# CasperTheCat/Vermilion

Measured on AMD Instinct MI355X. Metric: Mrays/sec (primary+secondary), 1920x1080 Sponza, higher is better.
Workload: dtype f32

## Files before the change

### vermilion_amd/csrc/api_render.inc

```
namespace {

Tuning make_tuning(const vmx_scene *sc, const vmx_opts *o) {
    Tuning tn;
    tn.refill_min = o->reserved[3] ? o->reserved[3] : 8u;
    tn.refill_primary = o->reserved[3] ? o->reserved[3] : 64u;
    tn.shade_min = o->reserved[4] ? o->reserved[4] : 16u;
    tn.leaf_min = 0xFFFFFFFFu;
    tn.sort_mode = o->reserved[5];
    tn.two_phase = false;
    tn.sorted = false;
    tn.bounce_records = false;
    tn.pool = false;
    tn.guide = false;
    const uint32_t cap = o->reserved[6];
    tn.lds_entries = std::min(sc->dev.stack_entries, cap ? cap : 10u);
    tn.lds_primary = std::min(sc->dev.stack_entries, cap ? cap : (uint32_t)VMX_LDS_PRIMARY);
    tn.lds_bounce = std::min(sc->dev.stack_entries, cap ? cap : 9u);
    tn.tail_threshold = o->reserved[2] ? o->reserved[2] : (16u << 20);
    return tn;
}


int bind_stack(vmx_scene *sc, const Tuning &tn, uint32_t entries, uint32_t grid, uint64_t items, WorkDev &wk, bool guided = false) {
    const uint64_t per_lane = items / ((uint64_t)grid * kPathsBlock);
// ... 248 lines not shown
    uint32_t smax = (uint32_t)std::max<uint64_t>(1, max_paths / npix);
    if (opts->samples_per_batch) smax = opts->samples_per_batch;
    smax = std::min(smax, fr.kmax);
    const size_t n_pad_cap = ((size_t)npix + 63u) & ~(size_t)63u;
    if (!opts->samples_per_batch && !legacy) {
        const size_t per_path = 16 + 64 + 8 + 16 + 12  + (sc->dev.tex ? 16 : 0) + (tn.sort_mode ? 12 : 0) + (fr.elide_dead ? 5 : 0) + 32 + (tn.guide ? 4 : 0) ;
        size_t free_b = 0, total_b = 0;
        HIP_TRY(hipMemGetInfo(&free_b, &total_b));
        const size_t held = ws.rayA.n + ws.state.n + ws.hit.n + ws.rad.n + ws.thr.n + (ws.ids[0].n + ws.ids[1].n + ws.ids[2].n) * 4 +
                            (ws.sort_keys[0].n + ws.sort_keys[1].n + ws.ids_sorted.n) * 4 + ws.out_rec.n + ws.live_ids.n * 4 +
                            ws.guide_fb.n * 4;
        job.mem_budget = (uint64_t)((free_b + held) / 10 * 9);
        if (const char *e = std::getenv("VMX_MEM_BUDGET_MB")) {
            const uint64_t cap = std::strtoull(e, nullptr, 10) << 20;
            if (cap) job.mem_budget = std::min(job.mem_budget, cap);
        }
        const uint64_t fixed = (uint64_t)npix * 48 + ((uint64_t)sc->n_inner * 512 + (uint64_t)sc->ntris * 64) + (64ull << 20);
        const uint64_t fit = job.mem_budget > fixed ? (job.mem_budget - fixed) / per_path : 0;
        const uint32_t s_fit = (uint32_t)std::min<uint64_t>(std::max<uint64_t>(1, fit / n_pad_cap), fr.kmax);
        if (s_fit < smax) smax = s_fit;
    }
    if (fr.early_stop) smax = std::min(smax, fr.nmin + 1 + (fr.quarter ? fr.kmax / fr.quarter - 1u : 0u));
    if (!fr.early_stop && !opts->samples_per_batch) {
        const uint32_t npass = (fr.kmax + smax - 1) / smax;
        smax = (fr.kmax + npass - 1) / npass;
    }
    job.smax = job.smax_alloc = smax;

    HIP_TRY((hipError_t)query_paths_blocks_per_cu(kPathsBlock, (kPathsBlock / 64) * (tn.lds_entries + 1) * 512, count, &job.rb, tn.guide));
    if (job.rb < 1) return fail(VMX_ERR_HIP, "kernel does not fit on a CU (LDS stack too deep?)");

    job.n_pad_max = (npix + 63u) & ~63u;
    const uint32_t tiles8_max = (((job.n_pad_max + sc->block - 1) / sc->block) + 7u) & ~7u;
    job.sub_cap = ((tiles8_max * smax) / kSubQueues + 2) * sc->block;
    job.sub_cap = job.sub_cap + job.sub_cap / 4 + 4096;
    tn.bounce_records = split_any && !tn.two_phase && !count && !tn.pool && fr.r2scale == 10.0f;
    if (split_any) {
        HIP_TRY((hipError_t)query_trace_q_blocks_per_cu(kPathsBlock, (kPathsBlock / 64) * (tn.lds_primary + 1) * 512, count, false,
                                                        tn.sorted, fr.elide_dead != 0, &job.tb));
        HIP_TRY((hipError_t)query_trace_q_blocks_per_cu(kPathsBlock, (kPathsBlock / 64) * (tn.lds_bounce + 1) * 512, count, true,
                                                        tn.sorted || tn.bounce_records, false, &job.tbb, tn.guide));
        if (job.tb < 1 || job.tbb < 1) return fail(VMX_ERR_HIP, "trace kernel does not fit on a CU");
        job.tbb = ab_bounce_blocks(job.tbb);
    }
    job.elide = split_any && fr.elide_dead;
    job.claims_on = split_any && !count && !job.elide && !(opts->reserved[0] & 0x800u) &&
                    (pipeline == 4 || (uint64_t)job.n_pad_max * smax >= kHybridPaths);
    job.fuse_on = job.claims_on && !tn.two_phase && !tn.sorted && !(opts->reserved[0] & 0x1000u);
    job.lists_on = job.claims_on && !(opts->reserved[0] & 0x2000u);
    job.live_words_max = ((size_t)job.n_pad_max * smax + 63) / 64;
    if (job.elide) job.live_tmp_bytes = live_compact_tmp_bytes((uint32_t)job.live_words_max);
    if (pixels->ensure(npix)) return fail(VMX_ERR_NOMEM, "hipMalloc failed for the per-pixel state");
    job.n_active = npix;
    return VMX_OK;
}

int render_init_pixels(vmx_scene *sc, RenderJob &job) {
    Workspace &ws = sc->ws;
    const uint32_t W = job.fr.width, rows = job.fr.local_rows;
    if (ws.order_w != W || ws.order_rows != rows) {
        tile_order(W, rows, ws.order);
        ws.order_w = W, ws.order_rows = rows;
    }
    HIP_TRY(hipMemcpyAsync(job.pixels->active[0].p, ws.order.data(), (size_t)job.npix * 4, hipMemcpyHostToDevice, job.s));
    LAUNCH_TRY(launch_init_pixels(PixelStateDev{job.pixels->accum.p, job.pixels->count.p, job.pixels->cursor.p}, job.npix, job.s));
    job.launches++;
    job.initialised = true;
    return VMX_OK;
}

constexpr uint32_t kClaimMinSamples = 64;
uint32_t claim_min_samples() {
#ifdef VMX_AB_KERNELS
    if (const char *e = std::getenv("VMX_CLAIM_MIN_SPP")) {
        const unsigned long v = std::strtoul(e, nullptr, 10);
        if (v) return (uint32_t)std::min<unsigned long>(v, 0xFFFFFFFFul);
    }
#endif
    return kClaimMinSamples;
}

int build_claims(vmx_scene *sc, const FrameDev &fr, const Tuning &tn, uint32_t npix, bool lists, hipStream_t s) {
    Workspace &ws = sc->ws;
    if (ws.claims.ensure((size_t)npix + 1)) return fail(VMX_ERR_NOMEM, "hipMalloc failed for the pixel claims");
    if (lists && ws.claim_lists.ensure((size_t)npix * kListWords)) return fail(VMX_ERR_NOMEM, "hipMalloc failed for the claim lists");
    WorkDev wk;
    std::memset(&wk, 0, sizeof(wk));
    wk.cam_inner = ws.cam_inner.p, wk.cam_tris = ws.cam_inner.p + std::max<size_t>(sc->n_inner, 1) * 64 * 8;
    const uint32_t tiles = ((fr.width + 7u) / 8u) * ((fr.local_rows + 7u) / 8u);
    LaunchCfg cfg = paths_cfg(sc, tn.lds_primary, (uint64_t)tiles * 64, 8);
    int rc = bind_stack(sc, tn, tn.lds_primary, cfg.grid, (uint64_t)tiles * 64, wk);
    if (rc) return rc;
    HIP_TRY(hipMemsetAsync(ws.claims.p + npix, 0, 4, s));
    LAUNCH_TRY(launch_pixel_claims(sc->dev, fr, wk, ws.claims.p, lists ? ws.claim_lists.p : nullptr, ws.claims.p + npix, cfg, s));
    return VMX_OK;
}

int nee_launch_cfg(vmx_scene *sc, const Tuning &tn, uint64_t items, bool rays, WorkDev &wk, LaunchCfg &cfg, bool budgeted = false) {
    int blocks = 0;
    HIP_TRY((hipError_t)query_nee_blocks_per_cu(kPathsBlock, (kPathsBlock / 64) * (tn.lds_entries + 1) * 512, rays, &blocks, budgeted));
    if (blocks < 1) return fail(VMX_ERR_HIP, "kernel does not fit on a CU (LDS stack too deep?)");
    cfg = paths_cfg(sc, tn.lds_entries, items, blocks);
    return bind_stack(sc, tn, tn.lds_entries, cfg.grid, items, wk);
}

int render_bind(vmx_scene *sc, RenderJob &job, uint32_t run_samples) {
    Workspace &ws = sc->ws;
    const FrameDev &fr = job.fr;
    const Tuning &tn = job.tn;
    const uint32_t smax = job.smax, n_pad_max = job.n_pad_max;
    hipStream_t s = job.s;
    if (job.nee) {
        if (ws.heads.ensure(kSubQueues * 32) || ws.rad.ensure((size_t)n_pad_max * smax * 16) || ws.next_count.ensure(32) ||
            ws.counters.ensure(1))
            return fail(VMX_ERR_NOMEM, "hipMalloc failed for the render workspace");
        job.px = PixelStateDev{job.pixels->accum.p, job.pixels->count.p, job.pixels->cursor.p};
        job.claims = job.claim_lists = nullptr;
        return VMX_OK;
    }
    if (job.split_any) {
        int rc = ensure_paths(sc, (size_t)n_pad_max * smax, job.pa, job.qi);
        if (rc == VMX_ERR_NOMEM && smax > 1 && !job.opts.samples_per_batch)
            return fail(VMX_ERR_NOMEM, "hipMalloc failed for the path arrays although " + std::to_string(job.mem_budget >> 20) +
                                           " MB were reported free: set VMX_MEM_BUDGET_MB or vmx_opts.reserved[1] (paths per pass)");
        if (rc) return rc;
    }
    else if (job.legacy) {
        int rc = ab_bind_legacy(sc, job);
        if (rc) return rc;
    }
    if (ws.heads.ensure(kSubQueues * 32)) return fail(VMX_ERR_NOMEM, "work heads");
    if (ws.rad_mask.ensure(((size_t)n_pad_max * smax + 63) / 64 + 8)) return fail(VMX_ERR_NOMEM, "hipMalloc failed for the radiance mask");
    if (job.split_any) job.pa.rad_mask = ws.rad_mask.p;
    if (job.split_any && tn.two_phase) {
        const size_t words = job.live_words_max + 2048;
        const size_t tmp = live_compact_tmp_bytes((uint32_t)words);
        if (ws.full_mask.ensure(words + 8) || ws.full_u32.ensure(2 * words + 16) || ws.full_tmp.ensure(tmp + 256))
            return fail(VMX_ERR_NOMEM, "hipMalloc failed for the two-phase shading lists");
        ws.full_words = words, ws.full_tmp_bytes = tmp;
    }
    if (job.split_any && (tn.sorted || tn.bounce_records)) {
        const size_t waves = (size_t)sc->num_cus * ((size_t)std::max(job.tb, job.tbb) + (tn.guide ? kGuideFallbackBlocks : 0u)) * (kPathsBlock / 64);
        ws.out_capacity = (size_t)n_pad_max * smax + waves * 256 + 1024;
        if (ws.out_capacity > 0xFFFFFFFFull) return fail(VMX_ERR_INVALID, "pass too large for the sorted ray records");
        if (ws.out_rec.ensure(ws.out_capacity * (tn.sorted ? 32 : 16)) || ws.out_count.ensure(32))
            return fail(VMX_ERR_NOMEM, "hipMalloc failed for the ray records");
    }
    if (job.split_any) {
        if (ws.guide_ctr.ensure(2) || (tn.guide && (ws.guide_fb.ensure((size_t)job.qi[0].sub_capacity * kSubQueues) ||
                                                    ws.guide_fb_count.ensure(32) || ws.guide_heads.ensure(32))))
            return fail(VMX_ERR_NOMEM, "hipMalloc failed for the guide tree's fallback list");
    }
    if (job.elide) {
        if (ws.live_mask.ensure(job.live_words_max + 8) || ws.live_u32.ensure(2 * job.live_words_max + 16) ||
            ws.live_ids.ensure((size_t)n_pad_max * smax + 64) || ws.live_tmp.ensure(job.live_tmp_bytes + 256))
            return fail(VMX_ERR_NOMEM, "hipMalloc failed for the live-path list");
    }
    if (ws.rad.ensure((size_t)n_pad_max * smax * 16) || ws.next_count.ensure(32) || ws.counters.ensure(1) ||
        (tn.guide && ws.guide_fused_ctr.ensure(2)))
        return fail(VMX_ERR_NOMEM, "hipMalloc failed for the render workspace");
    job.px = PixelStateDev{job.pixels->accum.p, job.pixels->count.p, job.pixels->cursor.p};
    if (job.split_any) {
        const size_t n_inner = std::max<size_t>(sc->n_inner, 1);
        if (ws.cam_inner.ensure(n_inner * 64 * 8 + (size_t)sc->ntris * 64))
            return fail(VMX_ERR_NOMEM, "hipMalloc failed for the camera tables");
        LAUNCH_TRY(launch_camera_tables(sc->dev, sc->n_inner, fr.px, fr.py, fr.pz, ws.cam_inner.p,
                                        ws.cam_inner.p + n_inner * 64 * 8, s));
        job.launches++;
    }
    job.claims = job.claim_lists = nullptr;
    if (job.claims_on) {
        uint32_t expect = fr.early_stop ? std::min(fr.kmax, fr.nmin + 1 + (fr.quarter ? fr.kmax / fr.quarter - 1u : 0u)) : fr.kmax;
        if (run_samples) expect = std::min(expect, run_samples);
        if (expect >= claim_min_samples()) {
            int rc = timed_begin(ws, job.timed, s, -1, VMX_K_OTHER);
            if (rc) return rc;
            if ((rc = build_claims(sc, fr, tn, job.npix, job.lists_on, s))) return rc;
// ... 639 lines not shown
```

### vermilion_amd/csrc/vmx_host.h

```cpp
namespace {

thread_local std::string g_err;

int fail(int code, const std::string &msg) {
    g_err = msg;
    return code;
}

#define HIP_TRY(expr)                                                                              \
    do {                                                                                           \
        hipError_t e_ = (expr);                                                                    \
        if (e_ != hipSuccess)                                                                      \
            return fail(VMX_ERR_HIP, std::string(#expr) + ": " + hipGetErrorString(e_));           \
    } while (0)

#define LAUNCH_TRY(expr)                                                                           \
    do {                                                                                           \
        int e_ = (expr);                                                                           \
        if (e_ != 0)                                                                               \
            return fail(VMX_ERR_HIP, std::string(#expr) + ": " + hipGetErrorString((hipError_t)e_)); \
    } while (0)

const vmx_sphere kReferenceSpheres[8] = {
    {{15.f, 140.f, 25.f}, 3.5f, {0.f * 15.f, .5f * 15.f, 1.0f * 15.f}, VMX_SPHERE_EMIT, {-55.f, 350.f, -150.f}, -1.f},
// ... 26 lines not shown
        if (p) (void)hipFree(p);
        p = nullptr;
        n = 0;
        hipError_t e = hipMalloc((void **)&p, std::max<size_t>(count, 1) * sizeof(T));
        if (e != hipSuccess) return (int)e;
        n = count;
        return 0;
    }
    void release() {
        if (p) (void)hipFree(p);
        p = nullptr;
        n = 0;
    }
};
static_assert(!std::is_copy_constructible<DevBuf<float>>::value, "DevBuf owns its memory: it moves, it is never copied");

struct NoCopy {
    NoCopy() = default;
    NoCopy(const NoCopy &) = delete;
    NoCopy &operator=(const NoCopy &) = delete;
};

struct DevStream : NoCopy {
    hipStream_t s = nullptr;
    ~DevStream() { if (s) (void)hipStreamDestroy(s); }
    operator hipStream_t() const { return s; }
};

struct EventPool : NoCopy {
    std::vector<hipEvent_t> ev;
    size_t used = 0;
    ~EventPool() { for (auto e : ev) (void)hipEventDestroy(e); }
    hipEvent_t get() {
        if (used == ev.size()) {
            hipEvent_t e;
            if (hipEventCreate(&e) != hipSuccess) return nullptr;
            ev.push_back(e);
        }
        return ev[used++];
    }
    void reset() { used = 0; }
};

struct Fence : NoCopy {
    hipEvent_t ev = nullptr;
    bool recorded = false;
    ~Fence() { if (ev) (void)hipEventDestroy(ev); }
    int wait(hipStream_t s) const {
        if (recorded) HIP_TRY(hipStreamWaitEvent(s, ev, 0));
        return VMX_OK;
    }
    int record(hipStream_t s) {
        if (!ev) HIP_TRY(hipEventCreateWithFlags(&ev, hipEventDisableTiming));
        HIP_TRY(hipEventRecord(ev, s));
        recorded = true;
        return VMX_OK;
    }
    int sync() const {
        if (recorded) HIP_TRY(hipEventSynchronize(ev));
        return VMX_OK;
    }
};

struct PixelBufs {
    DevBuf<unsigned char> accum;
    DevBuf<unsigned int> count, cursor, active[2];
    int ensure(size_t npix) {
        return accum.ensure(npix * 16) || count.ensure(npix) || cursor.ensure(npix) || active[0].ensure(npix) || active[1].ensure(npix);
    }
};

struct Workspace {
    DevBuf<unsigned char> queue_planes[2];
    DevBuf<unsigned int> queue_counts;
    DevBuf<unsigned int> heads;
    DevBuf<unsigned char> overflow_stack;
    DevBuf<unsigned char> rayA, state, hit, thr;
    DevBuf<unsigned int> ids[3], id_counts;
    DevBuf<unsigned int> sort_keys[2], ids_sorted;
    DevBuf<unsigned char> sort_tmp;
    DevBuf<unsigned char> cam_inner;
    DevBuf<unsigned int> claims;
    DevBuf<unsigned int> claim_lists;
    DevBuf<unsigned int> unclaimed, claimed_slots, unclaimed_u32;
    DevBuf<unsigned long long> unclaimed_mask;
    DevBuf<unsigned char> unclaimed_tmp;
    size_t unclaimed_words = 0, unclaimed_tmp_bytes = 0;
    DevBuf<unsigned int> walk_slots, walk_u32;
    DevBuf<unsigned long long> walk_mask;
    DevBuf<unsigned char> rad;
    DevBuf<unsigned long long> rad_mask;
    DevBuf<unsigned long long> live_mask;
    DevBuf<unsigned int> live_u32, live_ids;
    DevBuf<unsigned char> live_tmp;
    DevBuf<unsigned long long> full_mask;
    DevBuf<unsigned int> full_u32;
    DevBuf<unsigned char> full_tmp;
    size_t full_words = 0, full_tmp_bytes = 0;
    DevBuf<unsigned char> out_rec;
    DevBuf<unsigned int> out_count;
    size_t out_capacity = 0;
    DevBuf<unsigned int> guide_fb, guide_fb_count, guide_heads;
    DevBuf<unsigned long long> guide_ctr;
    DevBuf<unsigned long long> guide_fused_ctr;
    uint64_t guide_entries = 0;
    PixelBufs pixels;
    DevBuf<unsigned int> next_count;
    DevBuf<DevCounters> counters;
    DevBuf<float> out;
    std::vector<unsigned int> order;
    uint32_t order_w = 0, order_rows = 0;
    EventPool events;
};

}

#define VMX_OPAQUE __attribute__((visibility("hidden")))

struct vmx_scene {
    int device = 0;
    int num_cus = 0;
    DevStream stream;
    HostBvh bvh;
    LbvhDevice lbvh;
    bool device_built = false;
    uint32_t builder = VMX_BVH_REFERENCE;
    std::atomic<bool> flat_ready{true};
    bool flat_topology = true;
    uint32_t n_inner = 0;
    uint32_t ntris = 0, leaf_size = 4;
    std::vector<vmx_sphere> spheres;
    DevBuf<unsigned char> d_geom;
    DevBuf<AttrRecord> d_attrs;
    DevBuf<SphereDev> d_spheres;
    DevBuf<float> d_tex, d_tex1;
    uint32_t n_textures = 0;
    SceneDev dev{};
    std::mutex mu;
    Workspace ws;
    uint32_t block = 256;
    float bounds_lo[3] = {0, 0, 0}, bounds_hi[3] = {1, 1, 1};
    vmx_timings timings{};
    uint64_t fused_paths = 0;
    uint64_t list_settled = 0;
    uint64_t guide_settled = 0, guide_fallback = 0;
    uint64_t guide_entries = 0;
    uint64_t guide_fused_settled = 0, guide_fused_fallback = 0;
    struct VMX_OPAQUE Guide {
        std::shared_ptr<const HostBvh> host;
        const unsigned char *base = nullptr;
        uint32_t off = 0;
        size_t bytes = 0;
        uint32_t tri_off = 0, root_ref = 0, stack_entries = 0;
        float scene_max = 0.f;
        bool valid = false;
    } guide;
    struct QueryWs {
        DevBuf<unsigned int> head;
        DevBuf<unsigned char> overflow_stack;
        Fence done;
        uint32_t lds_entries = 0, overflow_entries = 0;
        uint32_t grid[2][kQueryModes] = {};
        uint32_t stack_entries = 0;
        DevBuf<unsigned char> albedo_rec;
    } qws;
    struct VMX_OPAQUE UpdateState {
// ... 213 lines not shown
```

### vermilion_amd/csrc/vmx_kernels.h

```cpp
#pragma once
#include <stdint.h>
#include "vmx_device.h"

namespace vmx {

constexpr uint32_t kSubQueues = 16;

struct QueueDev {
    void *planes;
    unsigned int *counts;
    uint32_t capacity;
    uint32_t sub_capacity;
};

struct PixelStateDev {
    void *accum;
    unsigned int *count;
    unsigned int *cursor;
};

struct PathArrays {
    void *rayA;
    void *state;
    void *hit;
// ... 58 lines not shown
    uint32_t fb_capacity;
    unsigned int *fb_ids;
    unsigned int *fb_count;
    unsigned long long *ctr;
    DevCounters *overflow;
};

struct GuidePathsDev {
    uint32_t off;
    uint32_t tri_off;
    uint32_t root_ref;
    float scene_max;
    unsigned long long *ctr;
};

struct QueryDev {
    const float *o, *d;
    const float *tmax;
    uint32_t n;
    uint32_t reserve;
    uint32_t refill_min;
    uint32_t lds_entries;
    uint32_t overflow_entries;
    uint32_t sample;
    void *overflow_stack;
    unsigned int *head;
    int32_t *tri_id;
    float *t;
    uint8_t *hit;
};

struct LaunchCfg {
    uint32_t grid;
    uint32_t block;
    uint32_t lds_bytes;
};

int launch_trace(const SceneDev &sc, const float *o, const float *d, uint32_t n, int32_t *tri_id,
                 float *t, DevCounters *counters, bool count, LaunchCfg cfg, void *stream);
int launch_raycast(const SceneDev &sc, const float *o, const float *d, uint32_t n, void *out_rayhit,
                   LaunchCfg cfg, void *stream);
int launch_primary_ids(const SceneDev &sc, const FrameDev &fr, uint32_t k, int32_t *tri_id, float *t,
                       LaunchCfg cfg, void *stream);

constexpr uint32_t kQueryCastRays = 3, kQueryCastCamera = 4, kQueryModes = 5;
int launch_query(const SceneDev &sc, const QueryDev &q, uint32_t mode, bool quad, LaunchCfg cfg, void *stream);
int query_query_blocks_per_cu(uint32_t block, uint32_t lds_bytes, uint32_t mode, bool quad, int *blocks);
int launch_raycast_query(const SceneDev &sc, const QueryDev &q, const FrameDev &fr, bool camera, bool quad, void *out,
                         LaunchCfg cfg, uint32_t finish_grid, void *stream);

struct RefitItem {
    uint32_t ref, dst;
};
constexpr uint32_t kRefitRoot = 0xFFFFFFFFu;
int launch_update_records(uint32_t ntris, const float *pos, const float *nrm, const float *uv, void *tris, void *attrs,
                          void *stream);
int launch_refit_level(const RefitItem *items, uint32_t n, const float *pos, const void *tris, void *inner,
                       float *root_box, void *stream);
int launch_attrs_by_id(uint32_t ntris, const void *tris, const void *attrs, float *nrm, float *uv, void *stream);

int launch_trig(const float *x, uint32_t n, float *cs, float *sn, void *stream);

int launch_init_pixels(PixelStateDev px, uint32_t npix, void *stream);
int launch_zero_u32(unsigned int *p, uint32_t n, void *stream);
#ifdef VMX_AB_KERNELS
int launch_primary(const SceneDev &sc, const FrameDev &fr, const unsigned int *active,
                   uint32_t n_active, uint32_t samples, PixelStateDev px, QueueDev qout, void *rad,
                   DevCounters *counters, bool count, bool loop_to_end, LaunchCfg cfg, void *stream);
int launch_radiance_init(const float *o, const float *d, uint32_t n, uint64_t seed, QueueDev qout,
                         void *stream);
int launch_bounce(const SceneDev &sc, float r2scale, uint32_t libm_double, QueueDev qin, uint32_t max_chunks, QueueDev qout,
                  void *rad, DevCounters *counters, bool count, bool loop_to_end, bool first_step,
                  LaunchCfg cfg, void *stream);
int query_blocks_per_cu(uint32_t block, uint32_t lds_bytes, bool count, int *primary_blocks, int *bounce_blocks);
int launch_trace_pool(const SceneDev &sc, const WorkDev &wk, PathArrays pa, LaunchCfg cfg, void *stream);
int query_trace_pool(uint32_t block, uint32_t pool_slots, uint32_t lds_levels, uint32_t *lds_bytes, int *blocks);
#endif
int launch_paths(const SceneDev &sc, const FrameDev &fr, const WorkDev &wk, PixelStateDev px, void *rad,
                 DevCounters *counters, bool count, LaunchCfg cfg, void *stream, const GuidePathsDev *guide = nullptr);
int query_paths_blocks_per_cu(uint32_t block, uint32_t lds_bytes, bool count, int *blocks, bool guide = false);
int launch_camera_tables(const SceneDev &sc, uint32_t n_inner, float ox, float oy, float oz, void *cam_inner,
                         void *cam_tris, void *stream);
int launch_pixel_claims(const SceneDev &sc, const FrameDev &fr, const WorkDev &wk, unsigned int *claims, unsigned int *lists, unsigned int *n_claimed,
                        LaunchCfg cfg, void *stream);
int launch_raygen(const SceneDev &sc, const FrameDev &fr, const WorkDev &wk, PixelStateDev px, PathArrays pa, void *stream);
int launch_raygen_live(const SceneDev &sc, const FrameDev &fr, const WorkDev &wk, PixelStateDev px, PathArrays pa, void *stream);
size_t live_compact_tmp_bytes(uint32_t nwords);
int launch_live_compact(const unsigned long long *live_mask, const unsigned int *live_cnt, uint32_t nwords,
                        unsigned int *offs, unsigned int *ids, unsigned int *count, void *tmp, size_t tmp_bytes, void *stream);
int launch_slot_lists(const unsigned long long *mask, const unsigned int *cnt, uint32_t nwords, uint32_t n_active, unsigned int *offs,
                      unsigned int *unclaimed, unsigned int *claimed, unsigned int *counts, void *tmp, size_t tmp_bytes, void *stream);
int launch_unclaimed_words(const unsigned int *active, uint32_t n_active, uint32_t n_pad, const unsigned int *claims,
                           unsigned long long *mask, unsigned int *cnt, void *stream);
int launch_walk_words(const unsigned int *active, uint32_t n_active, uint32_t n_pad, const unsigned int *claims,
                      const unsigned int *lists, unsigned long long *mask, unsigned int *cnt, void *stream);
int launch_trace_q(const SceneDev &sc, const FrameDev &fr, const WorkDev &wk, PixelStateDev px, PathArrays pa,
                   DevCounters *counters, bool count, bool from_queue, LaunchCfg cfg, void *stream, const GuideDev *guide = nullptr,
                   unsigned int *visits = nullptr);
int query_trace_q_blocks_per_cu(uint32_t block, uint32_t lds_bytes, bool count, bool from_queue, bool sorted, bool live, int *blocks,
                                bool guide = false);
int launch_shade(const SceneDev &sc, const FrameDev &fr, const WorkDev &wk, PixelStateDev px, PathArrays pa,
                 IdQueue qout, uint32_t max_chunks, DevCounters *counters, bool from_queue, void *stream);
int launch_shade_ends(const SceneDev &sc, const FrameDev &fr, const WorkDev &wk, PathArrays pa, unsigned long long *full_mask,
                      unsigned int *full_cnt, uint32_t max_chunks, DevCounters *counters, bool from_queue, void *stream);
int launch_tail(const SceneDev &sc, const FrameDev &fr, const WorkDev &wk, PathArrays pa, DevCounters *counters,
                bool count, LaunchCfg cfg, void *stream, const GuidePathsDev *guide = nullptr);
int launch_radiance_init_ids(const float *o, const float *d, uint32_t n, uint64_t seed, PathArrays pa,
                             IdQueue qout, void *stream);
int launch_resolve(const FrameDev &fr, const unsigned int *active, uint32_t n_active, uint32_t samples,
                   bool pixel_major, const void *rad, const unsigned long long *rad_mask, PixelStateDev px, unsigned int *next_active,
                   unsigned int *next_count, float *out_rgbaz, DevCounters *counters, void *stream, bool moments = false);
int launch_list_words(const unsigned int *list, uint32_t n, const unsigned char *select, const unsigned int *cursor, uint32_t kmax,
                      unsigned long long *mask, unsigned int *cnt, void *stream);
int launch_list_compact(const unsigned long long *mask, const unsigned int *cnt, uint32_t nwords, unsigned int *offs,
                        const unsigned int *src, unsigned int *dst, unsigned int *count, void *tmp, size_t tmp_bytes, void *stream);
struct SamplingPass {
    uint32_t width, height;
    uint32_t kmax, min_samples, radius;
    float threshold, floor;
    PixelStateDev px;
};
int launch_sampling_error(const SamplingPass &a, float *error, float *variance, void *stream);
int launch_sampling_select(const SamplingPass &a, unsigned char *select, unsigned int *count, void *stream);
int launch_bruteforce(const SceneDev &sc, const FrameDev &fr, const unsigned int *order, uint32_t npix, uint32_t flags,
                      float *out, DevCounters *counters, void *longs , unsigned int *long_count,
                      const WorkDev &stack , LaunchCfg cfg, void *stream);
int launch_bruteforce_long(const SceneDev &sc, const FrameDev &fr, uint32_t flags, float *out, DevCounters *counters,
                           const void *longs, const unsigned int *long_count, uint32_t count, const WorkDev &stack,
                           LaunchCfg cfg, void *stream);
int launch_preview(PixelStateDev px, uint32_t npix, uint32_t kmax, const float *finished, float *out_rgbaz, void *rgba8,
                   void *stream);
struct FilterSrc {
    const float *frame;
    PixelStateDev px;
    const float *finished;
    uint32_t kmax;
};
struct FilterPass {
    uint32_t width, height;
    uint32_t step;
    uint32_t squarings;
    float isc2, kz;
    const void *guide;
    FilterSrc src;
    const void *in_plane;
    void *out_plane;
    float *out_rgbaz;
    void *rgba8;
    bool first, last;
    float sl2;
    const void *albedo;
};
static_assert(sizeof(FilterPass) == 128, "FilterPass: a member moved (the kernels' argument offsets would)");
int launch_filter_guide(const void *rayhit, uint32_t npix, void *guide, void *stream);
int launch_atrous(const FilterPass &pass, void *stream);
int launch_demod_divide(const FilterPass &pass, void *stream);
int launch_variance_pack(const FilterPass &pass, const float *variance, void *stream);
int launch_atrous_var(const FilterPass &pass, void *stream);
struct UpsamplePass {
    uint32_t width, height, low_width, low_height;
    uint32_t squarings;
    float sigma_depth;
    const void *guide_low, *guide_full;
    const float *low;
    float *out_rgbaz;
    void *rgba8;
};
// ... 89 lines not shown
```

### vermilion_amd/csrc/vmx_kernels.hip

```cpp
#include <hip/hip_runtime.h>
#include <math.h>
#include <algorithm>
#include <stdint.h>

#include "vmx_kernels.h"
#include "pixel_claim.h"
#include "guide_walk.h"
#include <type_traits>

#ifndef VMX_CAM_BATCH
#define VMX_CAM_BATCH 16
#endif
#ifndef VMX_TRACE_WAVES_PER_SIMD
#define VMX_TRACE_WAVES_PER_SIMD 7
#endif


namespace vmx {
__device__ __forceinline__ float luminance(float r, float g, float b);
namespace {

constexpr float kInf = __builtin_huge_valf();

struct Cnt {
// ... 1369 lines not shown
            } else if ((int)cur < 0) {
                if (COUNT) {
                    if (P.depth == 0) c0.tris++;
                    else c1.tris++;
                }
                float dist;
                const bool hit = tri_test(q0, q1, q2.x, P.ox, P.oy, P.oz, P.dx, P.dy, P.dz, dist);
                if (hit && dist < best) {
                    if (GUIDE) second = best, cut = toff != 0 ? dist * kGwCut : dist;
                    best = dist;
                    slot = (int)(cur & kLeafStartMask);
                } else if (GUIDE && hit) {
                    second = fminf(second, dist);
                }
                cur = leaf_advance(cur);
            }
            if (cur == kPop) {
                const uint32_t ref = pop_to_next(stk, ovf, lds_entries, sp, GUIDE ? cut : best);
                cur = ref == kBottom ? kIdle : ref;
            }
        };
        if (__builtin_amdgcn_ballot_w64(exact && cur != kIdle) != 0) {
#pragma unroll 1
            for (int act = 0; act < 8; ++act) step(std::true_type{});
        } else {
#pragma unroll 1
            for (int act = 0; act < 8; ++act) step(std::false_type{});
        }
    }
    tally_flush<COUNT>(ctr, tl, c0, c1);
    if (GUIDE && lane == 0) {
        if (n_settled) atomicAdd(&gd.ctr[0], (unsigned long long)n_settled);
        if (n_fallback) atomicAdd(&gd.ctr[1], (unsigned long long)n_fallback);
    }
}





__global__ void k_camera_tables(SceneDev sc, uint32_t n_inner, float ox, float oy, float oz,
                                float4 *__restrict__ cam_inner, float4 *__restrict__ cam_tris) {
    const float4 *__restrict__ inner = (const float4 *)sc.inner;
    const float4 *__restrict__ tris = (const float4 *)sc.tris;
    const uint32_t total = n_inner + sc.ntris;
    for (uint32_t i = blockIdx.x * blockDim.x + threadIdx.x; i < total; i += gridDim.x * blockDim.x) {
        if (i < n_inner) {
            const float4 q0 = inner[i * 4], q1 = inner[i * 4 + 1], q2 = inner[i * 4 + 2], q3 = inner[i * 4 + 3];
            const float l0x = q0.x - ox, l0y = q0.y - oy, l0z = q0.z - oz, h0x = q0.w - ox, h0y = q1.x - oy, h0z = q1.y - oz;
            const float l1x = q1.z - ox, l1y = q1.w - oy, l1z = q2.x - oz, h1x = q2.y - ox, h1y = q2.z - oy, h1z = q2.w - oz;
            for (uint32_t o = 0; o < 8; ++o) {
                const bool sx = o & 1u, sy = o & 2u, sz = o & 4u;
                float4 *rec = cam_inner + ((size_t)o * n_inner + i) * 4;
                rec[0] = make_float4(sx ? h0x : l0x, sy ? h0y : l0y, sz ? h0z : l0z, sx ? l0x : h0x);
                rec[1] = make_float4(sy ? l0y : h0y, sz ? l0z : h0z, sx ? h1x : l1x, sy ? h1y : l1y);
                rec[2] = make_float4(sz ? h1z : l1z, sx ? l1x : h1x, sy ? l1y : h1y, sz ? l1z : h1z);
                rec[3] = q3;
            }
        } else {
            const uint32_t t = i - n_inner;
            const float4 a = tris[t * 3], b = tris[t * 3 + 1], c = tris[t * 3 + 2];
            const float e1x = a.w, e1y = b.x, e1z = b.y, e2x = b.z, e2y = b.w, e2z = c.x;
            const float tx = ox - a.x, ty = oy - a.y, tz = oz - a.z;
            float qx, qy, qz;
            cross3(tx, ty, tz, e1x, e1y, e1z, qx, qy, qz);
            const float cdot = dot3(e2x, e2y, e2z, qx, qy, qz);
            cam_tris[t * 4] = make_float4(e1x, e1y, e1z, e2x);
            cam_tris[t * 4 + 1] = make_float4(e2y, e2z, tx, ty);
            cam_tris[t * 4 + 2] = make_float4(tz, qx, qy, qz);
            cam_tris[t * 4 + 3] = make_float4(cdot, c.y, 0.f, 0.f);
        }
    }
}

struct ClaimStack {
    uint2 *stk, *ovf;
    int lds_entries;
    __device__ __forceinline__ void put(int i, uint32_t ref, float near) { stack_push(stk, ovf, lds_entries, i, make_uint2(ref, __float_as_uint(near))); }
    __device__ __forceinline__ void get(int i, uint32_t &ref, float &near) const {
        const uint2 e = stack_pop(stk, ovf, lds_entries, i);
        ref = e.x, near = __uint_as_float(e.y);
    }
};
__global__ void __launch_bounds__(256)
k_pixel_claims(SceneDev sc, FrameDev fr, const float *__restrict__ cam_inner, const float *__restrict__ cam_tris,
               unsigned int *__restrict__ claims, unsigned int *__restrict__ lists, unsigned int *n_claimed, uint32_t lds_levels,
               uint32_t overflow_entries, void *overflow_stack) {
    extern __shared__ uint2 lds_stack[];
    const uint32_t lane = threadIdx.x & 63u, wave = threadIdx.x >> 6;
    ClaimStack stk;
    stk.stk = lds_stack + (size_t)wave * (lds_levels + 1) * 64 + lane;
    stk.ovf = (uint2 *)overflow_stack + ((size_t)(blockIdx.x * (blockDim.x >> 6) + wave) * overflow_entries) * 64 + lane;
    stk.lds_entries = (int)lds_levels;
    PcFilm fm;
    for (int i = 0; i < 9; ++i) fm.m[i] = fr.m[i];
    fm.width = fr.width, fm.height = fr.height, fm.sensor_x = fr.sensor_x, fm.sensor_y = fr.sensor_y, fm.film_dist = fr.film_dist;
    const uint32_t tiles_x = (fr.width + 7u) / 8u, tiles = tiles_x * ((fr.local_rows + 7u) / 8u);
    uint32_t n = 0;
    for (uint32_t tile = blockIdx.x * (blockDim.x >> 6) + wave; tile < tiles; tile += gridDim.x * (blockDim.x >> 6)) {
        const uint32_t ty = tile / tiles_x, tx = tile - ty * tiles_x;
        const uint32_t x = tx * 8u + (lane & 7u), y = ty * 8u + (lane >> 3);
        if (x < fr.width && y < fr.local_rows) {
            const uint32_t lp = y * fr.width + x;
            uint32_t c;
            if (lists) {
                uint32_t l[kListWords];
                c = pc_pixel_claim_and_list(fm, global_pixel(fr, lp), cam_inner, cam_tris, sc.root_ref, stk,
                                            (int)(lds_levels + overflow_entries), l);
                ((uint4 *)lists)[lp] = make_uint4(l[0], l[1], l[2], l[3]);
            } else {
                c = pc_pixel_claim(fm, global_pixel(fr, lp), cam_inner, cam_tris, sc.root_ref, stk, (int)(lds_levels + overflow_entries));
            }
            claims[lp] = c;
            n += c != kClaimNone ? 1u : 0u;
        }
    }
    n = wave_sum(n);
    if (lane == 0 && n) atomicAdd(n_claimed, n);
}

__global__ void __launch_bounds__(256)
k_unclaimed_words(const unsigned int *__restrict__ active, uint32_t n_active, uint32_t n_pad, const unsigned int *__restrict__ claims,
                  unsigned long long *__restrict__ mask, unsigned int *__restrict__ cnt) {
    for (uint32_t s_idx = blockIdx.x * blockDim.x + threadIdx.x; s_idx < n_pad; s_idx += gridDim.x * blockDim.x) {
        const bool un = s_idx < n_active && claims[active[s_idx]] == kClaimNone;
        const unsigned long long bits = __builtin_amdgcn_ballot_w64(un);
        if ((threadIdx.x & 63u) == 0) mask[s_idx >> 6] = bits, cnt[s_idx >> 6] = (uint32_t)__popcll(bits);
    }
}

__global__ void __launch_bounds__(256)
k_walk_words(const unsigned int *__restrict__ active, uint32_t n_active, uint32_t n_pad, const unsigned int *__restrict__ claims,
             const unsigned int *__restrict__ lists, unsigned long long *__restrict__ mask, unsigned int *__restrict__ cnt) {
    for (uint32_t s_idx = blockIdx.x * blockDim.x + threadIdx.x; s_idx < n_pad; s_idx += gridDim.x * blockDim.x) {
        bool walk = false;
        if (s_idx < n_active) {
            const uint32_t lp = active[s_idx];
            walk = claims[lp] == kClaimNone && lists[(size_t)lp * kListWords] == kClaimNone;
        }
        const unsigned long long bits = __builtin_amdgcn_ballot_w64(walk);
        if ((threadIdx.x & 63u) == 0) mask[s_idx >> 6] = bits, cnt[s_idx >> 6] = (uint32_t)__popcll(bits);
    }
}

template <int LIVE, bool LISTS = false>
__global__ void __launch_bounds__(256)
k_raygen(SceneDev sc, FrameDev fr, WorkDev wk, PixelStateDev px, PathArrays pa) {
    static_assert(!LISTS || !LIVE, "list pixels are settled in the plain form");
    const uint32_t total = wk.samples * wk.n_pad;
    [[maybe_unused]] uint32_t n_listed = 0;
    if (wk.pixel_major && (wk.samples & 63u) == 0) {
        const uint32_t lane = threadIdx.x & 63u;
        const uint32_t waves = gridDim.x * (blockDim.x >> 6);
        const uint32_t chunks = wk.samples >> 6;
        const bool listed = !LIVE && wk.unclaimed != nullptr;
        const uint32_t units = listed ? *wk.unclaimed_count : wk.n_pad;
        for (uint32_t unit = (uint32_t)__builtin_amdgcn_readfirstlane((int)(blockIdx.x * (blockDim.x >> 6) + (threadIdx.x >> 6)));
             unit < units; unit += waves) {
            const uint32_t s_idx = listed ? wk.unclaimed[unit] : unit;
            const uint32_t pid_base = s_idx * wk.samples;
            if (s_idx < wk.n_active) {
                const uint32_t lp = wk.active[s_idx];
                const uint32_t pixel = global_pixel(fr, lp);
                const PixelKey pk = rng_pixel_key(fr.seed, pixel);
                const bool lights = (LIVE || fr.camera_bits) && pixel_may_reach_a_light(sc, fr, pixel);
                const uint32_t cur = px.cursor[lp];
                const uint32_t k0 = cur & ~kCursorStrided, kstep = (cur & kCursorStrided) ? fr.quarter : 1u;
                typedef uint32_t u32x4 __attribute__((ext_vector_type(4)));
                [[maybe_unused]] u32x4 lrec = {kClaimNone, kClaimNone, kClaimNone, kClaimNone};
                if constexpr (LISTS) lrec = ((const __attribute__((address_space(4))) u32x4 *)(uintptr_t)wk.claim_lists)[lp];
                for (uint32_t ch = 0; ch < chunks; ++ch) {
                    const uint32_t j = ch * 64u + lane;
                    const uint32_t k = (fr.lead != 0 && j >= fr.lead) ? (j - fr.lead + 1u) * fr.quarter : k0 + j * kstep;
                    bool live = false;
                    float dx = 0.f, dy = 0.f, dz = 0.f;
                    uint32_t depth = 0xFFFFFFFFu;
                    if (k < fr.kmax) {
                        Rng rng;
                        if (LIVE && !lights) {
                            rng_init_keyed(rng, pk, k);
                            (void)rng_next(rng);
                            (void)rng_next(rng);
                            live = step_bits<false>(sc, fr.r2scale, rng, 0, fr.px, fr.py, fr.pz, 0.f, 0.f, 0.f, 1.f, 1.f, 1.f, false) != 3u;
                        } else {
                            primary_ray_keyed(fr, pixel, pk, k, rng, dx, dy, dz);
                            if (LIVE) live = !step_is_dead<false>(sc, fr.r2scale, rng, 0, fr.px, fr.py, fr.pz, dx, dy, dz, 1.f, 1.f, 1.f);
                            else depth = fr.camera_bits ? step_bits<false>(sc, fr.r2scale, rng, 0, fr.px, fr.py, fr.pz, dx, dy, dz, 1.f, 1.f, 1.f, lights) : 0u;
                        }
                    }
                    if (!LIVE) ((float4 *)pa.rayA)[pid_base + j] = make_float4(dx, dy, dz, __uint_as_float(depth));
                    if (LIVE) {
                        const unsigned long long bits = __builtin_amdgcn_ballot_w64(live);
                        if (lane == 0) wk.live_mask[(pid_base >> 6) + ch] = bits, wk.live_cnt[(pid_base >> 6) + ch] = (uint32_t)__popcll(bits);
                    }
                    if constexpr (LISTS) {
                        if (lrec.x != kClaimNone) {
                            const float *ctris = (const float *)(const __attribute__((address_space(4))) float *)(uintptr_t)wk.cam_tris;
                            const bool has = depth != 0xFFFFFFFFu;
                            float t = 0.f;
                            uint32_t m = 0;
                            const bool settled = has && pc_list_settle(ctris, lrec.x, lrec.y, lrec.z, lrec.w, dx, dy, dz, t, m);
// ... 1270 lines not shown

int launch_init_pixels(PixelStateDev px, uint32_t npix, void *stream) {
    hipLaunchKernelGGL(k_init_pixels, dim3((npix + 255) / 256), dim3(256), 0, (hipStream_t)stream, px, npix);
    return launch_status();
}

int launch_zero_u32(unsigned int *p, uint32_t n, void *stream) {
    hipLaunchKernelGGL(k_zero_u32, dim3((n + 255) / 256), dim3(256), 0, (hipStream_t)stream, p, n);
    return launch_status();
}

int launch_paths(const SceneDev &sc, const FrameDev &fr, const WorkDev &wk, PixelStateDev px, void *rad,
                 DevCounters *counters, bool count, LaunchCfg cfg, void *stream, const GuidePathsDev *guide) {
    hipStream_t s = (hipStream_t)stream;
    dim3 g(cfg.grid), b(cfg.block);
#define VMX_GO(C, T) \
    hipLaunchKernelGGL((k_paths<C, 0, T>), g, b, cfg.lds_bytes, s, sc, fr, wk, px, (float4 *)rad, pa, counters)
    PathArrays pa{};
    if (guide && guide->off && !count) {
        if (sc.tex) hipLaunchKernelGGL((k_paths<false, 0, true, GuidePathsDev>), g, b, cfg.lds_bytes, s, sc, fr, wk, px, (float4 *)rad, pa, counters, *guide);
        else hipLaunchKernelGGL((k_paths<false, 0, false, GuidePathsDev>), g, b, cfg.lds_bytes, s, sc, fr, wk, px, (float4 *)rad, pa, counters, *guide);
    } else if (sc.tex) {
        if (count) VMX_GO(true, true);
        else VMX_GO(false, true);
    } else {
        if (count) VMX_GO(true, false);
        else VMX_GO(false, false);
    }
#undef VMX_GO
    return launch_status();
}

int launch_tail(const SceneDev &sc, const FrameDev &fr, const WorkDev &wk, PathArrays pa, DevCounters *counters,
                bool count, LaunchCfg cfg, void *stream, const GuidePathsDev *guide) {
    hipStream_t s = (hipStream_t)stream;
    dim3 g(cfg.grid), b(cfg.block);
    PixelStateDev px{nullptr, nullptr, nullptr};
#define VMX_GO(C, T) \
    hipLaunchKernelGGL((k_paths<C, 2, T>), g, b, cfg.lds_bytes, s, sc, fr, wk, px, (float4 *)pa.rad, pa, counters)
    if (guide && guide->off && !count) {
        if (sc.tex) hipLaunchKernelGGL((k_paths<false, 2, true, GuidePathsDev>), g, b, cfg.lds_bytes, s, sc, fr, wk, px, (float4 *)pa.rad, pa, counters, *guide);
        else hipLaunchKernelGGL((k_paths<false, 2, false, GuidePathsDev>), g, b, cfg.lds_bytes, s, sc, fr, wk, px, (float4 *)pa.rad, pa, counters, *guide);
    } else if (sc.tex) {
        if (count) VMX_GO(true, true);
        else VMX_GO(false, true);
    } else {
        if (count) VMX_GO(true, false);
        else VMX_GO(false, false);
    }
#undef VMX_GO
    return launch_status();
}

int launch_camera_tables(const SceneDev &sc, uint32_t n_inner, float ox, float oy, float oz, void *cam_inner,
                         void *cam_tris, void *stream) {
    const uint32_t total = n_inner + sc.ntris;
    uint32_t grid = std::min<uint32_t>((total + 255) / 256, 4096);
    if (grid == 0) grid = 1;
    hipLaunchKernelGGL(k_camera_tables, dim3(grid), dim3(256), 0, (hipStream_t)stream, sc, n_inner, ox, oy, oz,
                       (float4 *)cam_inner, (float4 *)cam_tris);
    return launch_status();
}

int launch_raygen(const SceneDev &sc, const FrameDev &fr, const WorkDev &wk, PixelStateDev px, PathArrays pa, void *stream) {
    const uint64_t total = (uint64_t)wk.samples * wk.n_pad;
    uint32_t grid = (uint32_t)std::min<uint64_t>((total + 255) / 256, 256u * 32u);
    if (grid == 0) grid = 1;
    if (wk.live_mask) hipLaunchKernelGGL(k_raygen<1>, dim3(grid), dim3(256), 0, (hipStream_t)stream, sc, fr, wk, px, pa);
    else if (wk.unclaimed && wk.claim_lists && wk.qids.ids) {
        if (!wk.pixel_major || (wk.samples & 63u) != 0 || !wk.cam_tris || !wk.list_ctr || !wk.qids.counts) return (int)hipErrorInvalidValue;
        hipLaunchKernelGGL((k_raygen<0, true>), dim3(grid), dim3(256), 0, (hipStream_t)stream, sc, fr, wk, px, pa);
    } else hipLaunchKernelGGL(k_raygen<0>, dim3(grid), dim3(256), 0, (hipStream_t)stream, sc, fr, wk, px, pa);
    return launch_status();
}

int launch_walk_words(const unsigned int *active, uint32_t n_active, uint32_t n_pad, const unsigned int *claims,
                      const unsigned int *lists, unsigned long long *mask, unsigned int *cnt, void *stream) {
    const uint32_t grid = std::max(1u, std::min<uint32_t>((n_pad + 255) / 256, 4096u));
    hipLaunchKernelGGL(k_walk_words, dim3(grid), dim3(256), 0, (hipStream_t)stream, active, n_active, n_pad, claims, lists, mask, cnt);
    return launch_status();
}

int launch_pixel_claims(const SceneDev &sc, const FrameDev &fr, const WorkDev &wk, unsigned int *claims, unsigned int *lists, unsigned int *n_claimed,
                        LaunchCfg cfg, void *stream) {
    hipLaunchKernelGGL(k_pixel_claims, dim3(cfg.grid), dim3(cfg.block), cfg.lds_bytes, (hipStream_t)stream, sc, fr,
                       (const float *)wk.cam_inner, (const float *)wk.cam_tris, claims, lists, n_claimed, wk.lds_entries, wk.overflow_entries,
                       wk.overflow_stack);
    return launch_status();
}

int launch_unclaimed_words(const unsigned int *active, uint32_t n_active, uint32_t n_pad, const unsigned int *claims,
                           unsigned long long *mask, unsigned int *cnt, void *stream) {
    const uint32_t grid = std::max(1u, std::min<uint32_t>((n_pad + 255) / 256, 4096u));
    hipLaunchKernelGGL(k_unclaimed_words, dim3(grid), dim3(256), 0, (hipStream_t)stream, active, n_active, n_pad, claims, mask, cnt);
    return launch_status();
}

int launch_raygen_live(const SceneDev &sc, const FrameDev &fr, const WorkDev &wk, PixelStateDev px, PathArrays pa, void *stream) {
    const uint64_t total = ((uint64_t)wk.samples * wk.n_pad + 2) / 3;
    uint32_t grid = (uint32_t)std::min<uint64_t>((total + 255) / 256, 256u * 32u);
    if (grid == 0) grid = 1;
    hipLaunchKernelGGL(k_raygen_live, dim3(grid), dim3(256), 0, (hipStream_t)stream, sc, fr, wk, px, pa);
    return launch_status();
}

using TraceWKernel = void (*)(SceneDev, FrameDev, WorkDev, PathArrays, GuideDev);
using TraceQKernel = void (*)(SceneDev, FrameDev, WorkDev, PixelStateDev, PathArrays, DevCounters *);
static TraceWKernel trace_w_kernel(bool from_queue, bool sorted, bool live, bool guide) {
    if (from_queue) {
        if (guide) {
            if (sorted) return k_trace_w<1, false, true, true>;
            return k_trace_w<1, false, false, true>;
        }
        if (sorted) return k_trace_w<1, false, true>;
        return k_trace_w<1>;
    }
    if (sorted) {
        if (live) return k_trace_w<0, true, true>;
        return k_trace_w<0, false, true>;
    }
    if (live) return k_trace_w<0, true>;
    return k_trace_w<0>;
}
static TraceQKernel trace_q_kernel(bool from_queue) {
    if (from_queue) return k_trace_q<true, 1>;
    return k_trace_q<true, 0>;
}

int launch_trace_q(const SceneDev &sc, const FrameDev &fr, const WorkDev &wk, PixelStateDev px, PathArrays pa,
                   DevCounters *counters, bool count, bool from_queue, LaunchCfg cfg, void *stream, const GuideDev *guide,
                   unsigned int *visits) {
    hipStream_t s = (hipStream_t)stream;
    dim3 g(cfg.grid), b(cfg.block);
    const bool guided = guide && guide->base && from_queue && !count;
    if (visits) {
        if (!guided || wk.out_rec) return (int)hipErrorInvalidValue;
        hipLaunchKernelGGL(k_trace_w_visits, g, b, cfg.lds_bytes, s, sc, fr, wk, pa, *guide, (uint2 *)visits);
        return launch_status();
    }
    GuideDev gd{};
    if (guided) gd = *guide;
    if (count) hipLaunchKernelGGL(trace_q_kernel(from_queue), g, b, cfg.lds_bytes, s, sc, fr, wk, px, pa, counters);
    else hipLaunchKernelGGL(trace_w_kernel(from_queue, wk.out_rec != nullptr, wk.live_ids != nullptr, guided), g, b, cfg.lds_bytes, s, sc, fr, wk, pa, gd);
    return launch_status();
}

int query_trace_q_blocks_per_cu(uint32_t block, uint32_t lds_bytes, bool count, bool from_queue, bool sorted, bool live, int *blocks,
                                bool guide) {
    int a = 0;
    const hipError_t e = count ? hipOccupancyMaxActiveBlocksPerMultiprocessor(&a, trace_q_kernel(from_queue), (int)block, lds_bytes)
                               : hipOccupancyMaxActiveBlocksPerMultiprocessor(&a, trace_w_kernel(from_queue, sorted, live, guide && from_queue), (int)block, lds_bytes);
    if (blocks) *blocks = a;
    return (int)e;
}

int launch_shade(const SceneDev &sc, const FrameDev &fr, const WorkDev &wk, PixelStateDev px, PathArrays pa,
                 IdQueue qout, uint32_t max_chunks, DevCounters *counters, bool from_queue, void *stream) {
    hipStream_t s = (hipStream_t)stream;
    const bool flat = wk.flat_ids != nullptr || wk.out_rec != nullptr;
    constexpr uint32_t kShadeGrid = 256u * VMX_SHADE_WPS;
    const bool dense = !from_queue && !flat && !wk.live_ids && wk.pixel_major && (wk.samples & 63u) == 0;
    const uint64_t items = flat ? kShadeGrid
                                : (from_queue ? (uint64_t)max_chunks * kSubQueues
                                              : (dense ? ((uint64_t)wk.n_pad + 3) / 4 : ((uint64_t)wk.samples * wk.n_pad + 255) / 256));
    uint32_t grid = (uint32_t)std::min<uint64_t>(items, kShadeGrid);
    if (grid == 0) grid = 1;
#define VMX_GO(S, T, E, Q, D)                                                                                                    \
    do {                                  \
        if (D && wk.fused) hipLaunchKernelGGL((k_shade<S, T, E, Q, D, D>), dim3(grid), dim3(256), 0, s, sc, fr, wk, px, pa, qout, max_chunks, counters); \
        else hipLaunchKernelGGL((k_shade<S, T, E, Q, D>), dim3(grid), dim3(256), 0, s, sc, fr, wk, px, pa, qout, max_chunks, counters); \
    } while (0)
// ... 143 lines not shown
```

Baseline: 12940.

## Split pixel claim and list building into compacted two-pass kernels

Pixel claims now use a cheap candidate pass that parks the candidate pair and ballots the pixels needing a full list walk. Those pixels are compacted with the existing live-compact scan and handled by a separate list kernel. Both kernels take work through atomic counters, and launch bounds and grid sizes now follow occupancy queries. The aim is to remove divergence, where a few expensive list walks stalled whole waves, and to balance load, at the cost of an extra launch, a scan and more workspace.

After: 13170 (median of 6 runs). +1.8%, better.

```diff
diff --git a/vermilion_amd/csrc/api_render.inc b/vermilion_amd/csrc/api_render.inc
--- a/vermilion_amd/csrc/api_render.inc
+++ b/vermilion_amd/csrc/api_render.inc
@@ -354,17 +354,42 @@
 
 int build_claims(vmx_scene *sc, const FrameDev &fr, const Tuning &tn, uint32_t npix, bool lists, hipStream_t s) {
     Workspace &ws = sc->ws;
-    if (ws.claims.ensure((size_t)npix + 1)) return fail(VMX_ERR_NOMEM, "hipMalloc failed for the pixel claims");
+    if (ws.claims.ensure((size_t)npix + 2)) return fail(VMX_ERR_NOMEM, "hipMalloc failed for the pixel claims");
     if (lists && ws.claim_lists.ensure((size_t)npix * kListWords)) return fail(VMX_ERR_NOMEM, "hipMalloc failed for the claim lists");
     WorkDev wk;
     std::memset(&wk, 0, sizeof(wk));
     wk.cam_inner = ws.cam_inner.p, wk.cam_tris = ws.cam_inner.p + std::max<size_t>(sc->n_inner, 1) * 64 * 8;
-    const uint32_t tiles = ((fr.width + 7u) / 8u) * ((fr.local_rows + 7u) / 8u);
-    LaunchCfg cfg = paths_cfg(sc, tn.lds_primary, (uint64_t)tiles * 64, 8);
-    int rc = bind_stack(sc, tn, tn.lds_primary, cfg.grid, (uint64_t)tiles * 64, wk);
-    if (rc) return rc;
-    HIP_TRY(hipMemsetAsync(ws.claims.p + npix, 0, 4, s));
-    LAUNCH_TRY(launch_pixel_claims(sc->dev, fr, wk, ws.claims.p, lists ? ws.claim_lists.p : nullptr, ws.claims.p + npix, cfg, s));
+    const uint64_t tiles = (uint64_t)((fr.width + 7u) / 8u) * ((fr.local_rows + 7u) / 8u);
+    if (tiles * 64 > 0xFFFFFFFFull) return fail(VMX_ERR_INVALID, "frame too large for the pixel claims");
+    int cblocks = 0;
+    HIP_TRY((hipError_t)query_pixel_claims_blocks_per_cu(kPathsBlock, (kPathsBlock / 64) * (tn.lds_primary + 1) * 512, &cblocks));
+    if (cblocks < 1) return fail(VMX_ERR_HIP, "kernel does not fit on a CU (LDS stack too deep?)");
+    LaunchCfg cfg = paths_cfg(sc, tn.lds_primary, tiles * 64, cblocks);
+    LaunchCfg lcfg = cfg;
+    size_t tmp_bytes = 0;
+    if (lists) {
+        int blocks = 0;
+        HIP_TRY((hipError_t)query_pixel_lists_blocks_per_cu(kPathsBlock, cfg.lds_bytes, &blocks));
+        if (blocks < 1) return fail(VMX_ERR_HIP, "kernel does not fit on a CU (LDS stack too deep?)");
+        lcfg = paths_cfg(sc, tn.lds_primary, (uint64_t)npix, blocks);
+        tmp_bytes = live_compact_tmp_bytes((uint32_t)tiles);
+        if (ws.claim_pend_mask.ensure(tiles) || ws.claim_pend_u32.ensure(2 * tiles + 2) || ws.claim_pend_ids.ensure(npix) ||
+            ws.claim_pend_tmp.ensure(tmp_bytes + 256))
+            return fail(VMX_ERR_NOMEM, "hipMalloc failed for the list of pixels without a claim");
+    }
+    int rc = bind_stack(sc, tn, tn.lds_primary, std::max(cfg.grid, lcfg.grid), tiles * 64, wk);
+    if (rc) return rc;
+    HIP_TRY(hipMemsetAsync(ws.claims.p + npix, 0, 8, s));
+    if (!lists) {
+        LAUNCH_TRY(launch_pixel_claims(sc->dev, fr, wk, ws.claims.p, nullptr, ws.claims.p + npix, nullptr, nullptr, cfg, s));
+    } else {
+        unsigned int *cnt = ws.claim_pend_u32.p, *offs = cnt + tiles, *len = offs + tiles, *head = len + 1;
+        LAUNCH_TRY(launch_pixel_claims(sc->dev, fr, wk, ws.claims.p, ws.claim_lists.p, ws.claims.p + npix, ws.claim_pend_mask.p, cnt, cfg, s));
+        HIP_TRY(hipMemsetAsync(len, 0, 8, s));
+        HIP_TRY((hipError_t)launch_live_compact(ws.claim_pend_mask.p, cnt, (uint32_t)tiles, offs, ws.claim_pend_ids.p, len,
+                                                ws.claim_pend_tmp.p, tmp_bytes, s));
+        LAUNCH_TRY(launch_pixel_lists(sc->dev, fr, wk, ws.claim_pend_ids.p, len, head, ws.claim_lists.p, lcfg, s));
+    }
     return VMX_OK;
 }
 
diff --git a/vermilion_amd/csrc/vmx_host.h b/vermilion_amd/csrc/vmx_host.h
--- a/vermilion_amd/csrc/vmx_host.h
+++ b/vermilion_amd/csrc/vmx_host.h
@@ -132,6 +132,9 @@
     DevBuf<unsigned char> cam_inner;
     DevBuf<unsigned int> claims;
     DevBuf<unsigned int> claim_lists;
+    DevBuf<unsigned long long> claim_pend_mask;
+    DevBuf<unsigned int> claim_pend_u32, claim_pend_ids;
+    DevBuf<unsigned char> claim_pend_tmp;
     DevBuf<unsigned int> unclaimed, claimed_slots, unclaimed_u32;
     DevBuf<unsigned long long> unclaimed_mask;
     DevBuf<unsigned char> unclaimed_tmp;
diff --git a/vermilion_amd/csrc/vmx_kernels.h b/vermilion_amd/csrc/vmx_kernels.h
--- a/vermilion_amd/csrc/vmx_kernels.h
+++ b/vermilion_amd/csrc/vmx_kernels.h
@@ -164,7 +164,11 @@
 int launch_camera_tables(const SceneDev &sc, uint32_t n_inner, float ox, float oy, float oz, void *cam_inner,
                          void *cam_tris, void *stream);
 int launch_pixel_claims(const SceneDev &sc, const FrameDev &fr, const WorkDev &wk, unsigned int *claims, unsigned int *lists, unsigned int *n_claimed,
-                        LaunchCfg cfg, void *stream);
+                        unsigned long long *pend_mask, unsigned int *pend_cnt, LaunchCfg cfg, void *stream);
+int launch_pixel_lists(const SceneDev &sc, const FrameDev &fr, const WorkDev &wk, const unsigned int *entries, const unsigned int *count,
+                       unsigned int *head, unsigned int *lists, LaunchCfg cfg, void *stream);
+int query_pixel_claims_blocks_per_cu(uint32_t block, uint32_t lds_bytes, int *blocks);
+int query_pixel_lists_blocks_per_cu(uint32_t block, uint32_t lds_bytes, int *blocks);
 int launch_raygen(const SceneDev &sc, const FrameDev &fr, const WorkDev &wk, PixelStateDev px, PathArrays pa, void *stream);
 int launch_raygen_live(const SceneDev &sc, const FrameDev &fr, const WorkDev &wk, PixelStateDev px, PathArrays pa, void *stream);
 size_t live_compact_tmp_bytes(uint32_t nwords);
diff --git a/vermilion_amd/csrc/vmx_kernels.hip b/vermilion_amd/csrc/vmx_kernels.hip
--- a/vermilion_amd/csrc/vmx_kernels.hip
+++ b/vermilion_amd/csrc/vmx_kernels.hip
@@ -1475,9 +1475,10 @@
         ref = e.x, near = __uint_as_float(e.y);
     }
 };
-__global__ void __launch_bounds__(256)
+__global__ void __launch_bounds__(256, 7)
 k_pixel_claims(SceneDev sc, FrameDev fr, const float *__restrict__ cam_inner, const float *__restrict__ cam_tris,
-               unsigned int *__restrict__ claims, unsigned int *__restrict__ lists, unsigned int *n_claimed, uint32_t lds_levels,
+               unsigned int *__restrict__ claims, unsigned int *__restrict__ lists, unsigned int *n_claimed,
+               unsigned long long *__restrict__ pend_mask, unsigned int *__restrict__ pend_cnt, uint32_t lds_levels,
                uint32_t overflow_entries, void *overflow_stack) {
     extern __shared__ uint2 lds_stack[];
     const uint32_t lane = threadIdx.x & 63u, wave = threadIdx.x >> 6;
@@ -1490,26 +1491,68 @@
     fm.width = fr.width, fm.height = fr.height, fm.sensor_x = fr.sensor_x, fm.sensor_y = fr.sensor_y, fm.film_dist = fr.film_dist;
     const uint32_t tiles_x = (fr.width + 7u) / 8u, tiles = tiles_x * ((fr.local_rows + 7u) / 8u);
     uint32_t n = 0;
-    for (uint32_t tile = blockIdx.x * (blockDim.x >> 6) + wave; tile < tiles; tile += gridDim.x * (blockDim.x >> 6)) {
+    for (;;) {
+        uint32_t tile = 0;
+        if (lane == 0) tile = atomicAdd(n_claimed + 1, 1u);
+        tile = (uint32_t)__builtin_amdgcn_readfirstlane((int)tile);
+        if (tile >= tiles) break;
         const uint32_t ty = tile / tiles_x, tx = tile - ty * tiles_x;
         const uint32_t x = tx * 8u + (lane & 7u), y = ty * 8u + (lane >> 3);
+        bool walks = false, claimed = false;
         if (x < fr.width && y < fr.local_rows) {
             const uint32_t lp = y * fr.width + x;
-            uint32_t c;
+            int cand, other;
+            const uint32_t c = pc_pixel_claim_cand(fm, global_pixel(fr, lp), cam_inner, cam_tris, sc.root_ref, stk,
+                                                   (int)(lds_levels + overflow_entries), cand, other);
             if (lists) {
-                uint32_t l[kListWords];
-                c = pc_pixel_claim_and_list(fm, global_pixel(fr, lp), cam_inner, cam_tris, sc.root_ref, stk,
-                                            (int)(lds_levels + overflow_entries), l);
-                ((uint4 *)lists)[lp] = make_uint4(l[0], l[1], l[2], l[3]);
-            } else {
-                c = pc_pixel_claim(fm, global_pixel(fr, lp), cam_inner, cam_tris, sc.root_ref, stk, (int)(lds_levels + overflow_entries));
+                walks = c == kClaimNone && cand >= -1;
+                ((uint4 *)lists)[lp] = walks ? make_uint4((uint32_t)cand, (uint32_t)other, kClaimNone, kClaimNone)
+                                             : make_uint4(kClaimNone, kClaimNone, kClaimNone, kClaimNone);
             }
             claims[lp] = c;
-            n += c != kClaimNone ? 1u : 0u;
-        }
-    }
-    n = wave_sum(n);
+            claimed = c != kClaimNone;
+        }
+        n += (uint32_t)__popcll(__builtin_amdgcn_ballot_w64(claimed));
+        if (lists) {
+            const unsigned long long bits = __builtin_amdgcn_ballot_w64(walks);
+            if (lane == 0) pend_mask[tile] = bits, pend_cnt[tile] = (uint32_t)__popcll(bits);
+        }
+    }
     if (lane == 0 && n) atomicAdd(n_claimed, n);
+}
+
+__global__ void __launch_bounds__(256, 5)
+k_pixel_lists(SceneDev sc, FrameDev fr, const float *__restrict__ cam_inner, const float *__restrict__ cam_tris,
+              const unsigned int *__restrict__ entries, const unsigned int *__restrict__ count, unsigned int *head,
+              unsigned int *__restrict__ lists, uint32_t lds_levels, uint32_t overflow_entries, void *overflow_stack) {
+    extern __shared__ uint2 lds_stack[];
+    const uint32_t lane = threadIdx.x & 63u, wave = threadIdx.x >> 6;
+    ClaimStack stk;
+    stk.stk = lds_stack + (size_t)wave * (lds_levels + 1) * 64 + lane;
+    stk.ovf = (uint2 *)overflow_stack + ((size_t)(blockIdx.x * (blockDim.x >> 6) + wave) * overflow_entries) * 64 + lane;
+    stk.lds_entries = (int)lds_levels;
+    PcFilm fm;
+    for (int i = 0; i < 9; ++i) fm.m[i] = fr.m[i];
+    fm.width = fr.width, fm.height = fr.height, fm.sensor_x = fr.sensor_x, fm.sensor_y = fr.sensor_y, fm.film_dist = fr.film_dist;
+    const uint32_t tiles_x = (fr.width + 7u) / 8u;
+    const uint32_t n = *count;
+    for (;;) {
+        uint32_t base = 0;
+        if (lane == 0) base = atomicAdd(head, 64u);
+        base = (uint32_t)__builtin_amdgcn_readfirstlane((int)base);
+        if (base >= n) break;
+        if (base + lane < n) {
+            const uint32_t e = entries[base + lane], tile = e >> 6;
+            const uint32_t ty = tile / tiles_x, tx = tile - ty * tiles_x;
+            const uint32_t lp = (ty * 8u + ((e & 63u) >> 3)) * fr.width + tx * 8u + (e & 7u);
+            uint4 *rec = (uint4 *)lists + lp;
+            const uint4 parked = *rec;
+            uint32_t l[kListWords];
+            pc_pixel_list(fm, global_pixel(fr, lp), cam_inner, cam_tris, sc.root_ref, stk, (int)(lds_levels + overflow_entries),
+                          (int)parked.x, (int)parked.y, l);
+            *rec = make_uint4(l[0], l[1], l[2], l[3]);
+        }
+    }
 }
 
 __global__ void __launch_bounds__(256)
@@ -2946,11 +2989,28 @@
 }
 
 int launch_pixel_claims(const SceneDev &sc, const FrameDev &fr, const WorkDev &wk, unsigned int *claims, unsigned int *lists, unsigned int *n_claimed,
-                        LaunchCfg cfg, void *stream) {
+                        unsigned long long *pend_mask, unsigned int *pend_cnt, LaunchCfg cfg, void *stream) {
+    if (lists && (!pend_mask || !pend_cnt)) return (int)hipErrorInvalidValue;
     hipLaunchKernelGGL(k_pixel_claims, dim3(cfg.grid), dim3(cfg.block), cfg.lds_bytes, (hipStream_t)stream, sc, fr,
-                       (const float *)wk.cam_inner, (const float *)wk.cam_tris, claims, lists, n_claimed, wk.lds_entries, wk.overflow_entries,
-                       wk.overflow_stack);
+                       (const float *)wk.cam_inner, (const float *)wk.cam_tris, claims, lists, n_claimed, pend_mask, pend_cnt,
+                       wk.lds_entries, wk.overflow_entries, wk.overflow_stack);
     return launch_status();
+}
+
+int launch_pixel_lists(const SceneDev &sc, const FrameDev &fr, const WorkDev &wk, const unsigned int *entries, const unsigned int *count,
+                       unsigned int *head, unsigned int *lists, LaunchCfg cfg, void *stream) {
+    hipLaunchKernelGGL(k_pixel_lists, dim3(cfg.grid), dim3(cfg.block), cfg.lds_bytes, (hipStream_t)stream, sc, fr,
+                       (const float *)wk.cam_inner, (const float *)wk.cam_tris, entries, count, head, lists, wk.lds_entries,
+                       wk.overflow_entries, wk.overflow_stack);
+    return launch_status();
+}
+
+int query_pixel_claims_blocks_per_cu(uint32_t block, uint32_t lds_bytes, int *blocks) {
+    return (int)hipOccupancyMaxActiveBlocksPerMultiprocessor(blocks, k_pixel_claims, (int)block, lds_bytes);
+}
+
+int query_pixel_lists_blocks_per_cu(uint32_t block, uint32_t lds_bytes, int *blocks) {
+    return (int)hipOccupancyMaxActiveBlocksPerMultiprocessor(blocks, k_pixel_lists, (int)block, lds_bytes);
 }
 
 int launch_unclaimed_words(const unsigned int *active, uint32_t n_active, uint32_t n_pad, const unsigned int *claims,
```
